# jayleicn/ClipBERT

Hardware: NVIDIA H100
Metric: clips/sec fwd+bwd MSRVTT ret (ResNet50+BERT-base) (higher is better)
Workload: dtype bf16

## Files before the change

clipbert_b200/csrc/common.cuh:

```cuda
#pragma once
#include <cuda.h>
#include <cuda_bf16.h>
#include <cuda_runtime.h>
#include <stdint.h>

#include "drop_cfg.h"

namespace cb {

#ifndef CB_SPIN_LIMIT
#define CB_SPIN_LIMIT (1u << 24)
#endif

__device__ __forceinline__ uint32_t smem_u32(const void* p) {
  return static_cast<uint32_t>(__cvta_generic_to_shared(p));
}

__device__ __forceinline__ void pdl_wait() { asm volatile("griddepcontrol.wait;" ::: "memory"); }
__device__ __forceinline__ void pdl_trigger() { asm volatile("griddepcontrol.launch_dependents;" ::: "memory"); }

__device__ __forceinline__ void mbar_init(uint64_t* bar, uint32_t count) {
  asm volatile("mbarrier.init.shared::cta.b64 [%0], %1;" ::"r"(smem_u32(bar)), "r"(count));
}
__device__ __forceinline__ void fence_mbar_init() {
// ... 94 lines not shown
  asm volatile("cp.async.bulk.wait_group.read %0;" ::"n"(N) : "memory");
}
template <int N>
__device__ __forceinline__ void tma_store_wait_all() {
  asm volatile("cp.async.bulk.wait_group %0;" ::"n"(N) : "memory");
}
__device__ __forceinline__ void named_bar_sync(uint32_t id, uint32_t nthreads) {
  asm volatile("bar.sync %0, %1;" ::"r"(id), "r"(nthreads) : "memory");
}
__device__ __forceinline__ void named_bar_arrive(uint32_t id, uint32_t nthreads) {
  asm volatile("bar.arrive %0, %1;" ::"r"(id), "r"(nthreads) : "memory");
}
template <uint32_t NREG>
__device__ __forceinline__ void setmaxnreg_dec() {
  asm volatile("setmaxnreg.dec.sync.aligned.u32 %0;" ::"n"(NREG));
}
template <uint32_t NREG>
__device__ __forceinline__ void setmaxnreg_inc() {
  asm volatile("setmaxnreg.inc.sync.aligned.u32 %0;" ::"n"(NREG));
}

__device__ __forceinline__ void wgmma_fence() { asm volatile("wgmma.fence.sync.aligned;" ::: "memory"); }
__device__ __forceinline__ void wgmma_commit() { asm volatile("wgmma.commit_group.sync.aligned;" ::: "memory"); }
template <int N>
__device__ __forceinline__ void wgmma_wait() {
  asm volatile("wgmma.wait_group.sync.aligned %0;" ::"n"(N) : "memory");
}
template <int R>
__device__ __forceinline__ void wgmma_fence_acc(float (&d)[R]) {
#pragma unroll
  for (int i = 0; i < R; ++i) asm volatile("" : "+f"(d[i])::"memory");
}

__device__ __forceinline__ uint64_t gmma_desc(uint32_t smem_addr, uint32_t lbo, uint32_t sbo) {
  uint64_t d = 0;
  d |= static_cast<uint64_t>((smem_addr & 0x3FFFFu) >> 4);
  d |= static_cast<uint64_t>((lbo >> 4) & 0x3FFFu) << 16;
  d |= static_cast<uint64_t>((sbo >> 4) & 0x3FFFu) << 32;
  d |= 1ull << 62;
  return d;
}

template <int TA, int TB>
__device__ __forceinline__ void wgmma_bf16_n64(float (&d)[32], uint64_t adesc, uint64_t bdesc, uint32_t accumulate) {
  asm volatile(
      "{\n\t.reg .pred p;\n\t"
      "setp.ne.b32 p, %34, 0;\n\t"
      "wgmma.mma_async.sync.aligned.m64n64k16.f32.bf16.bf16 "
      "{"
      "%0, %1, %2, %3, %4, %5, %6, %7, %8, %9, %10, %11, %12, %13, %14, %15, "
      "%16, %17, %18, %19, %20, %21, %22, %23, %24, %25, %26, %27, %28, %29, %30, %31"
      "}, %32, %33, p, 1, 1, %35, %36;\n\t}"
      : "+f"(d[0]), "+f"(d[1]), "+f"(d[2]), "+f"(d[3]), "+f"(d[4]), "+f"(d[5]), "+f"(d[6]), "+f"(d[7]),
        "+f"(d[8]), "+f"(d[9]), "+f"(d[10]), "+f"(d[11]), "+f"(d[12]), "+f"(d[13]), "+f"(d[14]), "+f"(d[15]),
        "+f"(d[16]), "+f"(d[17]), "+f"(d[18]), "+f"(d[19]), "+f"(d[20]), "+f"(d[21]), "+f"(d[22]), "+f"(d[23]),
        "+f"(d[24]), "+f"(d[25]), "+f"(d[26]), "+f"(d[27]), "+f"(d[28]), "+f"(d[29]), "+f"(d[30]), "+f"(d[31])
      : "l"(adesc), "l"(bdesc), "r"(accumulate), "n"(TA), "n"(TB));
}
template <int TA, int TB>
__device__ __forceinline__ void wgmma_bf16_n128(float (&d)[64], uint64_t adesc, uint64_t bdesc, uint32_t accumulate) {
  asm volatile(
      "{\n\t.reg .pred p;\n\t"
      "setp.ne.b32 p, %66, 0;\n\t"
      "wgmma.mma_async.sync.aligned.m64n128k16.f32.bf16.bf16 "
      "{"
      "%0, %1, %2, %3, %4, %5, %6, %7, %8, %9, %10, %11, %12, %13, %14, %15, "
      "%16, %17, %18, %19, %20, %21, %22, %23, %24, %25, %26, %27, %28, %29, %30, %31, "
      "%32, %33, %34, %35, %36, %37, %38, %39, %40, %41, %42, %43, %44, %45, %46, %47, "
      "%48, %49, %50, %51, %52, %53, %54, %55, %56, %57, %58, %59, %60, %61, %62, %63"
      "}, %64, %65, p, 1, 1, %67, %68;\n\t}"
      : "+f"(d[0]), "+f"(d[1]), "+f"(d[2]), "+f"(d[3]), "+f"(d[4]), "+f"(d[5]), "+f"(d[6]), "+f"(d[7]),
// ... 152 lines not shown
```

clipbert_b200/csrc/gemm.cu:

```cuda
#include <algorithm>

#include "common.cuh"
#include "host_util.h"

namespace cb {

constexpr int BM = 128;
constexpr int BK = 64;
constexpr int CONSUMER_WARPS = 8;
constexpr int GEMM_THREADS = (CONSUMER_WARPS + 1) * 32;
constexpr int PP_THREADS = 3 * 128;
constexpr int PP_PRODUCER_REGS = 40;
constexpr int PP_CONSUMER_REGS = 232;
constexpr int PP_BAR_TURN = 1;
constexpr int MAX_STAGES = 8;
constexpr int SMEM_LIMIT = 232448;
constexpr int STG_PITCH = 36;
constexpr int STG_WARP_FLOATS = 16 * STG_PITCH;
constexpr int EPI_BYTES = CONSUMER_WARPS * STG_WARP_FLOATS * 4;
constexpr int IN_BOX_BYTES = BM * 64 * 2;

struct GemmEpi {
  const float* scale;
  const float* shift;
// ... 219 lines not shown
    const int nch = min(KCH, n_iters - i);
    mbar_wait(&full_bar[s], ph);
    __syncwarp();
    wgmma_fence();
    wgmma_fence_acc(acc);
    for (int ch = 0; ch < nch; ++ch) {
      const uint32_t a_addr = smem0 + s * stage_bytes + ch * Cfg::STAGE_BYTES + wg * (64 * 128);
      const uint32_t b_addr = smem0 + s * stage_bytes + ch * Cfg::STAGE_BYTES + Cfg::A_BYTES;
#pragma unroll
      for (int k = 0; k < BK / 16; ++k) {
        const uint64_t ad = TA ? gmma_desc(a_addr + k * 2048, BK * 128, 1024) : gmma_desc(a_addr + k * 32, 16, 1024);
        const uint64_t bd = TB ? gmma_desc(b_addr + k * 2048, BK * 128, 1024) : gmma_desc(b_addr + k * 32, 16, 1024);
        wgmma_bf16<BN, TA, TB>(acc, ad, bd, (i > 0 || ch > 0 || k > 0) ? 1u : 0u);
      }
    }
    wgmma_commit();
    wgmma_wait<1>();
    wgmma_fence_acc(acc);
    if (prev >= 0) {
      __syncwarp();
      if (lane == 0) mbar_arrive(&empty_bar[prev]);
    }
    prev = s;
    if (++s == STAGES) { s = 0; ph ^= 1; }
  }
  wgmma_wait<0>();
  wgmma_fence_acc(acc);
  if (prev >= 0) {
    __syncwarp();
    if (lane == 0) mbar_arrive(&empty_bar[prev]);
  }
}

template <int BN, int TB>
__device__ __forceinline__ void mma_tile_pp(float (&acc)[2][BN / 2], uint32_t smem0, int stage_bytes, int KCH, int STAGES, int n_iters,
                                            int lane, int& s, uint32_t& ph, uint64_t* full_bar, uint64_t* empty_bar, int pass_bar,
                                            bool in_stage) {
  using Cfg = GemmCfg<BN>;
  int prev = -1;
  for (int i = 0; i < n_iters; i += KCH) {
    const int nch = min(KCH, n_iters - i);
    mbar_wait_unguarded(&full_bar[s], ph);
    __syncwarp();
    wgmma_fence();
    wgmma_fence_acc(acc[0]);
    wgmma_fence_acc(acc[1]);
    for (int ch = 0; ch < nch; ++ch) {
      const uint32_t a_addr = smem0 + s * stage_bytes + ch * Cfg::STAGE_BYTES;
      const uint32_t b_addr = a_addr + Cfg::A_BYTES;
#pragma unroll
      for (int k = 0; k < BK / 16; ++k) {
        const uint64_t bd = TB ? gmma_desc(b_addr + k * 2048, BK * 128, 1024) : gmma_desc(b_addr + k * 32, 16, 1024);
        const uint32_t accum = (i > 0 || ch > 0 || k > 0) ? 1u : 0u;
#pragma unroll
        for (int h = 0; h < 2; ++h) wgmma_bf16<BN, 0, TB>(acc[h], gmma_desc(a_addr + h * (64 * 128) + k * 32, 16, 1024), bd, accum);
      }
    }
    wgmma_commit();
    wgmma_wait<1>();
    wgmma_fence_acc(acc[0]);
    wgmma_fence_acc(acc[1]);
    if (prev >= 0) {
      __syncwarp();
      mbar_arrive_if(&empty_bar[prev], lane == 0);
    }
    prev = s;
    if (++s == STAGES) { s = 0; ph ^= 1; }
    if (pass_bar && i + KCH >= n_iters) {
      if (in_stage) mbar_wait_unguarded(&full_bar[s], ph);
      named_bar_arrive(pass_bar, 2 * 128);
    }
  }
  wgmma_wait<0>();
  wgmma_fence_acc(acc[0]);
  wgmma_fence_acc(acc[1]);
  if (prev >= 0) {
    __syncwarp();
    mbar_arrive_if(&empty_bar[prev], lane == 0);
  }
}

template <int BN, bool STORE = false>
__device__ __forceinline__ void wgrad_epilogue(const float (&acc)[BN / 2], float* obase, int64_t out_ld, const float* scale, int M, int N, int r0,
                                               int n0, int lane) {
  const int r1 = r0 + 8;
  const float rs0 = (r0 < M && scale) ? scale[r0] : 1.0f;
  const float rs1 = (r1 < M && scale) ? scale[r1] : 1.0f;
#pragma unroll
  for (int j = 0; j < BN / 8; ++j) {
    const int n = n0 + j * 8 + 2 * (lane & 3);
    if (n < N) {
      if constexpr (STORE) {
        if (r0 < M) *reinterpret_cast<float2*>(obase + static_cast<int64_t>(r0) * out_ld + n) = make_float2(acc[4 * j] * rs0, acc[4 * j + 1] * rs0);
        if (r1 < M) *reinterpret_cast<float2*>(obase + static_cast<int64_t>(r1) * out_ld + n) = make_float2(acc[4 * j + 2] * rs1, acc[4 * j + 3] * rs1);
      } else {
        if (r0 < M) red_add_f32x2(obase + static_cast<int64_t>(r0) * out_ld + n, acc[4 * j] * rs0, acc[4 * j + 1] * rs0);
        if (r1 < M) red_add_f32x2(obase + static_cast<int64_t>(r1) * out_ld + n, acc[4 * j + 2] * rs1, acc[4 * j + 3] * rs1);
      }
    }
  }
}

__device__ __forceinline__ uint32_t swz128(uint32_t box, int r, int q) { return box + r * 128 + ((q ^ (r & 7)) << 4); }

template <int BN, int MODE>
__global__ void __launch_bounds__(PP_THREADS, 1)
    gemm_pingpong_kernel(const __grid_constant__ CUtensorMap tmA, const __grid_constant__ CUtensorMap tmB, const __grid_constant__ CUtensorMap tmR,
                         const __grid_constant__ CUtensorMap tmX, int M, int N, int K, int ntaps, int tap_w, int tap_sign, int tiles_m,
                         int tiles_n, int total_tiles, int STAGES, int KCH, int N_IN, GemmEpi epi) {
  static_assert(MODE != 1 && BN <= 128, "TN / NN tiles of 128 x 64 or 128 x 128");
  using Cfg = GemmCfg<BN>;
  extern __shared__ uint8_t smem_raw[];
  uint8_t* smem = reinterpret_cast<uint8_t*>((reinterpret_cast<uintptr_t>(smem_raw) + 1023) & ~static_cast<uintptr_t>(1023));
  const int stage_bytes = KCH * Cfg::STAGE_BYTES;
  const bool has_res = epi.residual != nullptr, has_aux = epi.aux != nullptr;
  constexpr int IN_TILE_BYTES = (BN / 64) * IN_BOX_BYTES;
  const int in_bytes = (has_res + has_aux) * IN_TILE_BYTES;
  uint8_t* in_base = smem + STAGES * stage_bytes;
  uint8_t* stg_base = in_base + N_IN * in_bytes;
  uint64_t* full_bar = reinterpret_cast<uint64_t*>(stg_base + EPI_BYTES);
  uint64_t* empty_bar = full_bar + MAX_STAGES;
  uint64_t* in_full = empty_bar + MAX_STAGES;
  uint64_t* in_empty = in_full + 2;

  const int warp = __shfl_sync(0xffffffffu, static_cast<int>(threadIdx.x >> 5), 0);
  const int lane = threadIdx.x & 31;
  const int unit = blockIdx.x;
  const int n_units = gridDim.x;
  if (threadIdx.x == 0) dbg_stamp(epi, 0);
  pdl_trigger();
  if (threadIdx.x == 0) {
    tma_prefetch_desc(&tmA);
    tma_prefetch_desc(&tmB);
    if (has_res) tma_prefetch_desc(&tmR);
    if (has_aux) tma_prefetch_desc(&tmX);
    for (int s = 0; s < STAGES; ++s) {
      mbar_init(&full_bar[s], 1);
      mbar_init(&empty_bar[s], 4);
    }
    for (int b = 0; b < 2; ++b) {
      mbar_init(&in_full[b], 1);
      mbar_init(&in_empty[b], 4);
    }
    fence_mbar_init();
  }
  __syncthreads();
  const int kc_per_tap = (K + BK - 1) / BK;
  const int n_iters = ntaps * kc_per_tap;
  const bool in_stage = in_bytes && !N_IN;
  const int tile_stages = (n_iters + KCH - 1) / KCH + (in_stage ? 1 : 0);
  pdl_wait();
  if (threadIdx.x == 0) dbg_stamp(epi, 1);

  if (warp < 4) {
    setmaxnreg_dec<PP_PRODUCER_REGS>();
    if (warp == 0 && lane == 0) {
      constexpr int B_BOXES = (MODE == 0) ? 1 : BN / 64;
      int s = 0;
      uint32_t ph = 0;
      auto load_inputs = [&](int tile) {
        const TileInfo t = decode_tile<BN>(tile, tiles_m, tiles_n);
        uint64_t* bar;
        uint8_t* dst;
        if (N_IN) {
          const int local = (tile - unit) / n_units;
          const int b = N_IN == 2 ? (local & 1) : 0;
          const int uses = N_IN == 2 ? (local >> 1) : local;
          mbar_wait(&in_empty[b], (static_cast<uint32_t>(uses) & 1u) ^ 1u);
          bar = &in_full[local & 1];
          dst = in_base + b * in_bytes;
        } else {
          mbar_wait(&empty_bar[s], ph ^ 1);
          bar = &full_bar[s];
          dst = smem + s * stage_bytes;
          if (++s == STAGES) { s = 0; ph ^= 1; }
        }
        mbar_expect_tx(bar, in_bytes);
        if (has_res) {
#pragma unroll
          for (int j = 0; j < BN / 64; ++j) tma_load_2d(dst + j * IN_BOX_BYTES, &tmR, bar, t.n0 + j * 64, t.m0);
          dst += IN_TILE_BYTES;
        }
        if (has_aux) {
#pragma unroll
          for (int j = 0; j < BN / 64; ++j) tma_load_2d(dst + j * IN_BOX_BYTES, &tmX, bar, t.n0 + j * 64, t.m0);
        }
      };
      int pend = -1;
      for (int tile = unit; tile < total_tiles; tile += n_units) {
        const TileInfo t = decode_tile<BN>(tile, tiles_m, tiles_n);
        const bool inputs_first = tile < unit + N_IN * n_units;
        if (in_bytes && N_IN && inputs_first) load_inputs(tile);
        for (int i = 0; i < n_iters; i += KCH) {
          const int nch = min(KCH, n_iters - i);
          mbar_wait(&empty_bar[s], ph ^ 1);
          mbar_expect_tx(&full_bar[s], nch * Cfg::STAGE_BYTES);
          int tp = 0, kc = i;
          if (ntaps > 1) { tp = i / kc_per_tap; kc = i - tp * kc_per_tap; }
          for (int ch = 0; ch < nch; ++ch) {
            uint8_t* sa = smem + s * stage_bytes + ch * Cfg::STAGE_BYTES;
            uint8_t* sb = sa + Cfg::A_BYTES;
            int shift = 0;
            if (ntaps == 9) shift = tap_sign * ((tp / 3 - 1) * tap_w + (tp % 3 - 1));
            else if (ntaps > 1) shift = tap_sign * tp * tap_w;
            tma_load_2d(sa, &tmA, &full_bar[s], kc * BK, t.m0 + shift);
            if (MODE == 0) {
              tma_load_2d(sb, &tmB, &full_bar[s], tp * K + kc * BK, t.n0);
            } else if (epi.mn3d) {
              tma_load_3d(sb, &tmB, &full_bar[s], 0, kc * BK, (tp * N + t.n0) >> 6);
            } else {
#pragma unroll
              for (int j = 0; j < B_BOXES; ++j) tma_load_2d(sb + j * (BK * 128), &tmB, &full_bar[s], tp * N + t.n0 + j * 64, kc * BK);
            }
            if (++kc == kc_per_tap) { kc = 0; ++tp; }
          }
          if (++s == STAGES) { s = 0; ph ^= 1; }
          if (i == 0 && tile == unit) dbg_stamp(epi, 2);
        }
        if (in_stage) load_inputs(tile);
        if (pend >= 0) load_inputs(pend);
        pend = (in_bytes && N_IN && !inputs_first) ? tile : -1;
      }
      if (pend >= 0) load_inputs(pend);
      dbg_stamp(epi, 3);
    }
    return;
  }

  setmaxnreg_inc<PP_CONSUMER_REGS>();
  const int wg = (warp >> 2) - 1;
  const int wq = warp & 3;
  const uint32_t smem0 = smem_u32(smem);
  const uint64_t dseed = epi.drop_thresh ? drop_seed(epi.seed, epi.seed_off) : 0ull;
  float acc[2][BN / 2];
  int s = 0;
  uint32_t ph = 0;
  auto ring_skip = [&](int n) {
    s += n;
    while (s >= STAGES) { s -= STAGES; ph ^= 1; }
  };
  if (wg == 1) ring_skip(tile_stages);

  const int er = lane & 15, eh = lane >> 4;
  float* stg = reinterpret_cast<float*>(stg_base) + (warp - 4) * STG_WARP_FLOATS;
  const bool has_out2 = epi.out2 != nullptr;
  const bool has_shift = epi.shift != nullptr;
  const bool full = (N & 15) == 0 && epi.scale == nullptr;
  const bool drop = epi.drop_thresh != 0;
  int kind = EK_GENERIC;
  if (full) {
    if (!drop && !has_out2 && !has_aux && (epi.act == CB_ACT_NONE || epi.act == CB_ACT_RELU)) kind = EK_SHIFT_ACT;
    else if (!drop && !has_out2 && !has_shift && has_aux && epi.aux_mode == CB_AUX_RELU_MASK && epi.act == CB_ACT_NONE) kind = EK_RELU_MASK;
    else if (drop && !has_out2 && !has_aux && epi.act == CB_ACT_NONE) kind = EK_DROP_RES;
    else if (!drop && has_out2 && !has_aux && !has_res && epi.act == CB_ACT_GELU_STASH_GRAD) kind = EK_GELU_STASH;
    else if (!drop && !has_out2 && !has_shift && has_aux && epi.aux_mode == CB_AUX_MUL && epi.act == CB_ACT_NONE) kind = EK_AUX_MUL;
  }
  const bool kind_relu = epi.act == CB_ACT_RELU;
  const bool guard = (N & 15) != 0;

  for (int local = wg, tile = unit + wg * n_units; tile < total_tiles; local += 2, tile += 2 * n_units) {
    const TileInfo t = decode_tile<BN>(tile, tiles_m, tiles_n);
    if (local > 0) named_bar_sync(PP_BAR_TURN + wg, 2 * 128);
    const int pass = tile + n_units < total_tiles ? PP_BAR_TURN + (wg ^ 1) : 0;
    mma_tile_pp<BN, MODE != 0>(acc, smem0, stage_bytes, KCH, STAGES, n_iters, lane, s, ph, full_bar, empty_bar, pass, in_stage);

    const uint32_t in_buf = N_IN ? smem_u32(in_base) + (N_IN == 2 ? wg : 0) * in_bytes : smem0 + s * stage_bytes;
    if (in_bytes) {
      if (N_IN) mbar_wait_unguarded(&in_full[wg], static_cast<uint32_t>(local >> 1) & 1u);
      else mbar_wait_unguarded(&full_bar[s], ph);
    }
    int orow_half[2];
#pragma unroll
    for (int h = 0; h < 2; ++h) {
      const int m = t.m0 + h * 64 + wq * 16 + er;
      bool row_ok = m < M;
      int64_t orow = m;
      if (epi.rowmap == CB_ROWMAP_PAD) {
        const int hw = epi.H * epi.W;
        const int img = m / hw;
        const int r = m - img * hw;
        const int y = r / epi.W, x = r - y * epi.W;
        orow = (static_cast<int64_t>(img) * (epi.H + 2) + y + 1) * (epi.W + 2) + x + 1;
      } else if (epi.rowmap == CB_ROWMAP_UNPAD) {
        const int wp = epi.W + 2, hp = epi.H + 2;
        const int img = m / (hp * wp);
        const int r = m - img * (hp * wp);
        const int y = r / wp, x = r - y * wp;
        row_ok = row_ok && y >= 1 && y <= epi.H && x >= 1 && x <= epi.W;
        orow = (static_cast<int64_t>(img) * epi.H + (y - 1)) * epi.W + (x - 1);
      }
      orow_half[h] = row_ok ? static_cast<int>(orow) : -1;
    }
#pragma unroll
    for (int sc = 0; sc < BN / 32; ++sc) {
#pragma unroll 1
      for (int h = 0; h < 2; ++h) {
        const int wrow = h * 64 + wq * 16;
// ... 83 lines not shown
    }
    if (in_bytes) {
      __syncwarp();
      if (lane == 0) mbar_arrive(N_IN ? &in_empty[N_IN == 2 ? wg : 0] : &empty_bar[s]);
      if (!N_IN && ++s == STAGES) { s = 0; ph ^= 1; }
    }
    ring_skip(tile_stages);
  }
  if (threadIdx.x == 4 * 32) dbg_stamp(epi, 11);
}

static int g_sm_limit = 0;
static int sm_count_device() {
  static int n = 0;
  if (n == 0) {
    int dev = 0;
    cudaGetDevice(&dev);
    cudaDeviceGetAttribute(&n, cudaDevAttrMultiProcessorCount, dev);
    if (n <= 0) n = 132;
  }
  return n;
}
static int sm_count() {
  const int n = sm_count_device();
  return (g_sm_limit > 0 && g_sm_limit < n) ? g_sm_limit : n;
}
static int plan_sm_count() { return g_det.load(std::memory_order_relaxed) ? sm_count_device() : sm_count(); }

static long long* g_gemm_timeline = nullptr;
static int g_mn3d = 1;


struct SmemPlan {
  int epi_bytes, kch, stages, chunk_bytes, n_in;
};
static SmemPlan plan_ring(int bn, bool staging, int kiters, int force_kch, int in_bytes, int n_in) {
  SmemPlan p;
  const int limit = SMEM_LIMIT;
  p.chunk_bytes = BM * BK * 2 + bn * BK * 2;
  p.epi_bytes = staging ? EPI_BYTES : 0;
  p.n_in = n_in;
  const int chunks_fit = (limit - 1024 - GemmCfg<64>::BAR_BYTES - p.epi_bytes - n_in * in_bytes) / p.chunk_bytes;
  const int min_stages = kiters > chunks_fit ? 3 : 2;
  p.kch = 1;
  if (force_kch > 0) p.kch = force_kch;
  else if (kiters >= 4 && chunks_fit >= 4 * min_stages) p.kch = 4;
  else if (kiters >= 2 && chunks_fit >= 2 * min_stages) p.kch = 2;
  if (p.kch > kiters) p.kch = kiters;
  if (p.kch > 1 && chunks_fit / p.kch < 2) p.kch = 1;
  p.stages = chunks_fit / p.kch;
  if (p.stages > MAX_STAGES) p.stages = MAX_STAGES;
  const int stage_iters = ceil_div(kiters, p.kch);
  const int cap = staging ? 2 * stage_iters + 1 : (stage_iters + 1 > 2 ? stage_iters + 1 : 2);
  if (p.stages > cap) p.stages = cap;
  return p;
}
static SmemPlan plan_smem(int bn, bool staging, int kiters, int force_kch = 0, int in_bytes = 0) {
  const SmemPlan none = plan_ring(bn, staging, kiters, force_kch, 0, 0);
  if (in_bytes == 0) return none;
  const SmemPlan two = plan_ring(bn, staging, kiters, force_kch, in_bytes, 2);
  if (two.stages >= 2 && two.stages * two.kch >= kiters) return two;
  if (kiters > 4 && none.stages >= 2 && none.kch * none.chunk_bytes >= in_bytes) return none;
  return plan_ring(bn, staging, kiters, force_kch, in_bytes, 1);
}
static int epi_in_bytes(const cb_gemm_desc& d, int bn) {
  return d.mode == CB_GEMM_WGRAD ? 0 : ((d.residual != nullptr) + (d.aux != nullptr)) * (bn / 64) * IN_BOX_BYTES;
}

static int real_splits(int kc, int want) {
  const int sp = want < 1 ? 1 : (want > kc ? kc : want);
  return ceil_div(kc, ceil_div(kc, sp));
}

struct SplitReduceJob {
  float* out;
  const float* ws;
  int64_t out_ld;
  int M, W, S;
};
struct SplitReduce {
  int njobs;
  SplitReduceJob j[8];
};
__global__ void __launch_bounds__(256) wgrad_split_reduce_kernel(const __grid_constant__ SplitReduce r) {
  pdl_wait();
  pdl_trigger();
  const SplitReduceJob& J = r.j[blockIdx.y];
  const int w4 = J.W / 4;
  const int64_t total = static_cast<int64_t>(J.M) * w4, plane = static_cast<int64_t>(J.M) * J.W;
  for (int64_t i = static_cast<int64_t>(blockIdx.x) * 256 + threadIdx.x; i < total; i += static_cast<int64_t>(gridDim.x) * 256) {
    const int64_t m = i / w4;
    const int c = static_cast<int>(i - m * w4) * 4;
    float4* o = reinterpret_cast<float4*>(J.out + m * J.out_ld + c);
    float4 v = *o;
    const float* p = J.ws + m * J.W + c;
    for (int s = 0; s < J.S; ++s) {
      const float4 a = *reinterpret_cast<const float4*>(p + s * plane);
      v.x += a.x; v.y += a.y; v.z += a.z; v.w += a.w;
    }
    *o = v;
  }
}
static int launch_split_reduce(const SplitReduce& r, cudaStream_t stream, const char* what) {
  int64_t most = 0;
  for (int i = 0; i < r.njobs; ++i) most = std::max(most, static_cast<int64_t>(r.j[i].M) * (r.j[i].W / 4));
  const int gx = static_cast<int>(std::min<int64_t>(1024, (most + 255) / 256));
  launch_k(wgrad_split_reduce_kernel, dim3(gx, r.njobs), 256, 0, stream, r);
  return check_launch(what);
}

template <int BN, int MODE>
static int launch_gemm(const cb_gemm_desc& d, const GemmEpi& epi_in, cudaStream_t stream) {
  GemmEpi epi = epi_in;
  using Cfg = GemmCfg<BN>;
  static bool attr_set = false;
  auto kern = gemm_pingpong_kernel<BN, MODE>;
  if (!attr_set) {
    cudaError_t e = cudaFuncSetAttribute(kern, cudaFuncAttributeMaxDynamicSharedMemorySize, SMEM_LIMIT);
    if (e != cudaSuccess) {
      set_error("cudaFuncSetAttribute(smem=%d): %s", SMEM_LIMIT, cudaGetErrorString(e));
      return CB_ERR_CUDA;
    }
    attr_set = true;
  }
  alignas(64) CUtensorMap ta, tb, tr, tx;
  bool mn3d = false;
  const int tiles_m = ceil_div(d.m, BM), tiles_n = ceil_div(d.n, BN);
  const int total = tiles_m * tiles_n;
  const int kiters = ceil_div(d.k, BK) * d.ntaps;
  bool ok = get_tmap_2d(&ta, d.a, d.k, d.a_rows, d.a_ld, BK, BM);
  if (MODE == 0) {
    ok = ok && get_tmap_2d(&tb, d.b, static_cast<uint64_t>(d.k) * d.ntaps, d.b_rows, d.b_ld, BK, BN);
  } else {
    mn3d = g_mn3d && d.n % 64 == 0 &&
           get_tmap_3d_mn(&tb, d.b, static_cast<uint64_t>(d.n) * d.ntaps, d.b_rows, d.b_ld, BK, BN / 64);
    if (!mn3d) ok = ok && get_tmap_2d(&tb, d.b, static_cast<uint64_t>(d.n) * d.ntaps, d.b_rows, d.b_ld, 64, BK);
  }
  tr = ta;
  tx = ta;
  if (d.residual) ok = ok && get_tmap_2d(&tr, d.residual, d.n, d.m, d.res_ld, 64, BM);
  if (d.aux) ok = ok && get_tmap_2d(&tx, d.aux, d.n, d.m, d.aux_ld, 64, BM);
  if (!ok) return CB_ERR_CUDA;
  epi.mn3d = mn3d ? 1 : 0;
  const int units = sm_count();
  const int grid = total < units ? total : units;
  const int in_bytes = epi_in_bytes(d, BN);
  const SmemPlan sp = plan_smem(BN, true, kiters, (d.reserved >> 8) & 15, in_bytes);
  const int kch = sp.kch, stages = sp.stages;
  if (stages < 2) {
    set_error("cb_gemm: not enough shared memory for a 2-stage pipeline (BN=%d, epilogue %d B + inputs %d B)", BN, sp.epi_bytes,
              in_bytes);
    return CB_ERR_INVALID;
  }
  const int smem_bytes = stages * kch * Cfg::STAGE_BYTES + sp.n_in * in_bytes + sp.epi_bytes + Cfg::BAR_BYTES + 1024;
  launch_gemm_k(kern, grid, PP_THREADS, smem_bytes, stream, ta, tb, tr, tx, d.m, d.n, d.k, d.ntaps, d.tap_w, d.tap_sign, tiles_m,
                tiles_n, total, stages, kch, sp.n_in, epi);
  return check_launch("cb_gemm");
}

struct LaunchCfg {
  int bn, splits;
};

static LaunchCfg choose_config(const cb_gemm_desc& d, int units) {
  const int kc = ceil_div(d.k, BK);
  const bool wgrad = d.mode == CB_GEMM_WGRAD;
  const int block_n = (!wgrad && d.block_n == 256) ? 128 : d.block_n;
  static const int cand[3] = {64, 128, 256};
  LaunchCfg best = {64, 1};
  double best_cost = 1e30;
  for (int c = 0; c < 3; ++c) {
    const int bn = cand[c];
    if (block_n && bn != block_n) continue;
    if (!wgrad && bn == 256) continue;
    if (bn > 64 && d.n <= bn / 2) continue;
    const int64_t base = static_cast<int64_t>(ceil_div(d.m, BM)) * ceil_div(d.n, bn) * (wgrad ? d.ntaps : 1);
    const int max_split = wgrad ? (d.split_k > 0 ? d.split_k : (kc < 32 ? kc : 32)) : 1;
    for (int sp = (wgrad && d.split_k > 0) ? d.split_k : 1; sp <= max_split; ++sp) {
      const int ips = ceil_div(wgrad ? kc : kc * d.ntaps, sp);
      const int real_sp = wgrad ? ceil_div(kc, ips) : 1;
      const int64_t tiles = base * real_sp;
      const double rounds = static_cast<double>((tiles + units - 1) / units);
      const SmemPlan pl = plan_smem(bn, !wgrad, ips, (d.reserved >> 8) & 15, epi_in_bytes(d, bn));
      if (pl.stages < 2) continue;
      const double shallow = (pl.stages * pl.kch < 3 && ips > 2) ? 3.0 : 1.0;
      const double stage_cost = 450.0 + pl.kch * pl.chunk_bytes / 60.0;
      const double main_loop = ceil_div(ips, pl.kch) * stage_cost * shallow;
      double cost;
      if (wgrad) {
        cost = rounds * (main_loop + bn * 24.0) + 2500.0;
      } else {
        const double epi = bn * 30.0;
        const double per_tile = main_loop > 0.5 * (main_loop + epi) ? main_loop : 0.5 * (main_loop + epi);
        cost = rounds * per_tile + 0.5 * epi + 2500.0;
      }
      if (cost < best_cost) {
        best_cost = cost;
        best = {bn, real_sp};
      }
    }
  }
  return best;
}

constexpr int WG_MAX_PROBLEMS = 8;
struct WgradProblem {
  CUtensorMap tmA, tmB;
  float* out;
  const float* scale;
  int64_t out_ld;
  int M, N, K;
  int ntaps, tap_w, tap_sign;
  int iters_per_split, tiles_m, tiles_n;
  int tile_begin;
  int mn3d;
};
struct WgradGroup {
  int nprob, total_tiles;
  WgradProblem p[WG_MAX_PROBLEMS];
};
// ... 211 lines not shown
  return bytes;
}

static int check_wgrad_desc(const cb_gemm_desc& d, const char* who) {
  CB_REQUIRE(d.mode == CB_GEMM_WGRAD && d.out_fp32 == 1, "%s: not an fp32 WGRAD descriptor", who);
  CB_REQUIRE(d.a && d.b && d.out && d.m > 0 && d.n > 0 && d.k > 0, "%s: null operand / empty shape", who);
  CB_REQUIRE(d.m % 8 == 0 && d.n % 8 == 0, "%s: m, n must be multiples of 8 (got %d, %d)", who, d.m, d.n);
  CB_REQUIRE(d.out_ld % 4 == 0, "%s: out_ld must be a multiple of 4", who);
  CB_REQUIRE((reinterpret_cast<uintptr_t>(d.out) & 15) == 0, "%s: out must be 16-byte aligned", who);
  CB_REQUIRE(d.ntaps == 1 || d.ntaps == 9, "%s: ntaps must be 1 or 9 (got %d)", who, d.ntaps);
  return CB_OK;
}

static int launch_wgrad(const cb_gemm_desc* descs, int n, int bn, int splits, cudaStream_t stream, const char* what) {
  int64_t need = 0;
  if (g_det.load(std::memory_order_relaxed))
    for (int i = 0; i < n; ++i) need += wgrad_ws_bytes(descs[i], real_splits(ceil_div(descs[i].k, BK), splits));
  const cb_gemm_desc& d0 = descs[0];
  CB_REQUIRE(need == 0 || (d0.workspace != nullptr && d0.workspace_bytes >= need && (reinterpret_cast<uintptr_t>(d0.workspace) & 15) == 0),
             "%s: deterministic mode needs a 16-byte aligned workspace of %lld bytes in descs[0] (%s_workspace_bytes), got %lld", what,
             static_cast<long long>(need), what, static_cast<long long>(d0.workspace ? d0.workspace_bytes : 0));
  float* ws = static_cast<float*>(d0.workspace);
  switch (bn) {
    case 64: return need ? launch_wgrad_group<64, true>(descs, n, splits, ws, stream, what)
                         : launch_wgrad_group<64, false>(descs, n, splits, ws, stream, what);
    case 128: return need ? launch_wgrad_group<128, true>(descs, n, splits, ws, stream, what)
                          : launch_wgrad_group<128, false>(descs, n, splits, ws, stream, what);
    case 256: return need ? launch_wgrad_group<256, true>(descs, n, splits, ws, stream, what)
                          : launch_wgrad_group<256, false>(descs, n, splits, ws, stream, what);
    default: set_error("%s: block_n must be 0, 64, 128 or 256 (got %d)", what, bn); return CB_ERR_INVALID;
  }
}

}

extern "C" void cb_debug_gemm_timeline(void* device_buf) { cb::g_gemm_timeline = static_cast<long long*>(device_buf); }
extern "C" void cb_debug_gemm_mn3d(int on) { cb::g_mn3d = on ? 1 : 0; }
extern "C" void cb_debug_gemm_occ2(int, double) {}
extern "C" void cb_debug_gemm_sm_limit(int n) { cb::g_sm_limit = n > 0 ? n : 0; }

extern "C" int cb_gemm(const cb_gemm_desc* dp, void* stream_v) {
  using namespace cb;
  CB_REQUIRE(dp != nullptr, "cb_gemm: null descriptor");
  const cb_gemm_desc& d = *dp;
  cudaStream_t stream = static_cast<cudaStream_t>(stream_v);
  CB_REQUIRE(d.a && d.b && d.out, "cb_gemm: null operand pointer");
  CB_REQUIRE(d.m > 0 && d.n > 0 && d.k > 0, "cb_gemm: empty problem m=%d n=%d k=%d", d.m, d.n, d.k);
  CB_REQUIRE(d.ntaps == 1 || d.ntaps == 9 || (d.ntaps == 4 && d.mode == CB_GEMM_TN),
             "cb_gemm: ntaps must be 1, 9 (3x3 conv) or 4 (row taps, TN only) (got %d)", d.ntaps);
  CB_REQUIRE(d.mode == CB_GEMM_TN || d.mode == CB_GEMM_WGRAD || d.mode == CB_GEMM_NN, "cb_gemm: bad mode %d", d.mode);
  CB_REQUIRE(d.dropout_p >= 0.0f && d.dropout_p <= 1.0f, "cb_gemm: dropout_p %g outside [0, 1]", d.dropout_p);

  GemmEpi epi;
  epi.scale = d.scale;
  epi.shift = d.shift;
  epi.residual = static_cast<const __nv_bfloat16*>(d.residual);
  epi.aux = static_cast<const __nv_bfloat16*>(d.aux);
  epi.aux_mode = d.aux ? d.aux_mode : CB_AUX_NONE;
  epi.act = d.act;
  epi.out = d.out;
  epi.out_ld = d.out_ld;
  epi.out_fp32 = d.out_fp32;
  epi.out2 = static_cast<__nv_bfloat16*>(d.out2);
  epi.out2_ld = d.out2_ld;
  epi.rowmap = d.rowmap;
  epi.H = d.map_h;
  epi.W = d.map_w;
  epi.seed = d.dropout_seed;
  epi.dbg = g_gemm_timeline;
  epi.mn3d = 0;
  {
    const DropCfg dc = make_drop(d.dropout_p, d.dropout_seed);
// ... 72 lines not shown
```

include/clipbert_b200.h:

```cpp
#ifndef CLIPBERT_B200_H_
#define CLIPBERT_B200_H_

#include <stddef.h>
#include <stdint.h>

#ifdef __cplusplus
extern "C" {
#endif

typedef enum cb_status {
  CB_OK = 0,
  CB_ERR_INVALID = -1,
  CB_ERR_CUDA = -2,
  CB_ERR_UNSUPPORTED = -3
} cb_status;

const char* cb_last_error(void);
int cb_version(void);
int cb_sm_arch(void);
int64_t cb_launch_count(void);
int cb_set_pdl(int enable);

int cb_set_deterministic(int enable);

// ... 23 lines not shown
  int32_t m, n, k;
  const void* a;
  int64_t a_rows, a_ld;
  const void* b;
  int64_t b_rows, b_ld;
  int32_t ntaps, tap_w, tap_sign;
  int32_t split_k;
  const float* scale;
  const float* shift;
  const void* residual;
  int64_t res_ld;
  const void* aux;
  int64_t aux_ld;
  int32_t aux_mode;
  int32_t act;
  void* out;
  int64_t out_ld;
  int32_t out_fp32;
  void* out2;
  int64_t out2_ld;
  int32_t rowmap, map_h, map_w;
  float dropout_p;
  uint64_t dropout_seed;
  int32_t block_n;
  int32_t reserved;
  void* workspace;
  int64_t workspace_bytes;
} cb_gemm_desc;

int cb_gemm(const cb_gemm_desc* desc, void* stream);
int64_t cb_gemm_workspace_bytes(const cb_gemm_desc* desc);
int cb_gemm_wgrad_group(const cb_gemm_desc* descs, int n, void* stream);
int64_t cb_gemm_wgrad_group_workspace_bytes(const cb_gemm_desc* descs, int n);

int cb_layernorm_fwd(const void* x, const float* gamma, const float* beta, void* y, float* stats, int m, int hidden,
                     float eps, void* stream);
int cb_layernorm_bwd(const void* dy, const void* x, const float* stats, const float* gamma, void* dx, void* dx_drop,
                     float* dgamma, float* dbeta, float* dbias_drop, int m, int hidden, float dropout_p,
                     uint64_t dropout_seed, void* stream);
int64_t cb_layernorm_bwd_scratch_bytes(int m);
int cb_layernorm_bwd_det(const void* dy, const void* x, const float* stats, const float* gamma, void* dx, void* dx_drop,
                         float* dgamma, float* dbeta, float* dbias_drop, int m, int hidden, float dropout_p,
                         uint64_t dropout_seed, float* scratch, int64_t scratch_bytes, void* stream);

int cb_embed_text_fwd(const int64_t* ids, const float* word, const float* pos, const float* type0, const float* gamma,
                      const float* beta, void* out, float* stats, int nseq, int lt, int l, int vocab, int hidden,
                      float eps, float dropout_p, uint64_t seed, void* stream);
int cb_embed_text_bwd(const void* dh, const int64_t* ids, const float* word, const float* pos, const float* type0,
                      const float* gamma, const float* stats, float* dword, float* dpos, float* dtype0, float* dgamma,
                      float* dbeta, int nseq, int lt, int l, int vocab, int hidden, float dropout_p, uint64_t seed,
                      void* stream);
int cb_embed_visual_fwd(const void* grid, const int32_t* seq2vid, int n_ex, const float* rowemb, const float* colemb,
                        const float* type0, const float* gamma, const float* beta, void* out, float* stats, int nseq,
                        int t, int gh, int gw, int lt, int l, int hidden, float eps, float dropout_p, uint64_t seed,
                        void* stream);
int cb_embed_visual_bwd(const void* dh, const void* grid, const int32_t* seq2vid, const int32_t* vid_start, int n_ex,
                        const float* rowemb, const float* colemb, const float* type0, const float* gamma,
                        const float* stats, float* dv_tmp, void* dgrid, float* drow, float* dcol, float* dtype0,
                        float* dgamma, float* dbeta, int nseq, int nvid, int t, int gh, int gw, int lt, int l, int hidden,
                        float dropout_p, uint64_t seed, void* stream);
int64_t cb_embed_text_bwd_scratch_bytes(int nseq, int lt);
int cb_embed_text_bwd_det(const void* dh, const int64_t* ids, const float* word, const float* pos, const float* type0,
                          const float* gamma, const float* stats, float* dword, float* dpos, float* dtype0, float* dgamma,
                          float* dbeta, int nseq, int lt, int l, int vocab, int hidden, float dropout_p, uint64_t seed,
                          float* scratch, int64_t scratch_bytes, void* stream);
int64_t cb_embed_visual_bwd_scratch_bytes(int nseq, int gh, int gw);
// ... 66 lines not shown
```

Measured before the change: 3984.

## Reuse a shared-memory halo slab across the nine taps of 3x3 conv GEMMs

For 3x3 implicit-GEMM convolutions in the TN ping-pong kernel, each output tile now loads the activation rows plus a halo once into a double-buffered shared-memory slab. All nine taps then read their A operand by offsetting the wgmma descriptor into that slab, instead of reloading a shifted A tile per tap through the stage ring. This is meant to cut TMA and L2 traffic and shrink each ring stage to B only. In exchange the slab takes shared memory and pipeline depth, and the path depends on 128B-swizzle descriptors staying valid at arbitrary row offsets. The planner falls back to the old path when fewer than three stages fit, and a debug kernel is added to check swizzle row-phase behaviour.

After: 3984 (median of 6 runs). Within noise of the previous version (-0.0%).

```diff
diff --git a/clipbert_b200/csrc/common.cuh b/clipbert_b200/csrc/common.cuh
--- a/clipbert_b200/csrc/common.cuh
+++ b/clipbert_b200/csrc/common.cuh
@@ -150,11 +150,12 @@
   for (int i = 0; i < R; ++i) asm volatile("" : "+f"(d[i])::"memory");
 }
 
-__device__ __forceinline__ uint64_t gmma_desc(uint32_t smem_addr, uint32_t lbo, uint32_t sbo) {
+__device__ __forceinline__ uint64_t gmma_desc(uint32_t smem_addr, uint32_t lbo, uint32_t sbo, uint32_t base_offset = 0) {
   uint64_t d = 0;
   d |= static_cast<uint64_t>((smem_addr & 0x3FFFFu) >> 4);
   d |= static_cast<uint64_t>((lbo >> 4) & 0x3FFFu) << 16;
   d |= static_cast<uint64_t>((sbo >> 4) & 0x3FFFu) << 32;
+  d |= static_cast<uint64_t>(base_offset & 7u) << 49;
   d |= 1ull << 62;
   return d;
 }
diff --git a/clipbert_b200/csrc/gemm.cu b/clipbert_b200/csrc/gemm.cu
--- a/clipbert_b200/csrc/gemm.cu
+++ b/clipbert_b200/csrc/gemm.cu
@@ -275,12 +275,14 @@
   }
 }
 
-template <int BN, int TB>
-__device__ __forceinline__ void mma_tile_pp(float (&acc)[2][BN / 2], uint32_t smem0, int stage_bytes, int KCH, int STAGES, int n_iters,
-                                            int lane, int& s, uint32_t& ph, uint64_t* full_bar, uint64_t* empty_bar, int pass_bar,
-                                            bool in_stage) {
+template <int BN, int TB, bool SLAB>
+__device__ __forceinline__ void mma_tile_pp(float (&acc)[2][BN / 2], uint32_t smem0, int stage_bytes, int chunk_bytes, int KCH, int STAGES,
+                                            int n_iters, int lane, int& s, uint32_t& ph, uint64_t* full_bar, uint64_t* empty_bar,
+                                            int pass_bar, bool in_stage, uint32_t slab, int slab_pitch, int kc_per_tap, int tap_w,
+                                            int tap_sign) {
   using Cfg = GemmCfg<BN>;
   int prev = -1;
+  int tp = 0, kc = 0;
   for (int i = 0; i < n_iters; i += KCH) {
     const int nch = min(KCH, n_iters - i);
     mbar_wait_unguarded(&full_bar[s], ph);
@@ -289,8 +291,13 @@
     wgmma_fence_acc(acc[0]);
     wgmma_fence_acc(acc[1]);
     for (int ch = 0; ch < nch; ++ch) {
-      const uint32_t a_addr = smem0 + s * stage_bytes + ch * Cfg::STAGE_BYTES;
-      const uint32_t b_addr = a_addr + Cfg::A_BYTES;
+      uint32_t a_addr = smem0 + s * stage_bytes + ch * chunk_bytes;
+      uint32_t b_addr = a_addr + Cfg::A_BYTES;
+      if constexpr (SLAB) {
+        b_addr = a_addr;
+        a_addr = slab + kc * slab_pitch + (tap_sign * ((tp / 3 - 1) * tap_w + (tp % 3 - 1)) + tap_w + 1) * 128;
+        if (++kc == kc_per_tap) { kc = 0; ++tp; }
+      }
 #pragma unroll
       for (int k = 0; k < BK / 16; ++k) {
         const uint64_t bd = TB ? gmma_desc(b_addr + k * 2048, BK * 128, 1024) : gmma_desc(b_addr + k * 32, 16, 1024);
@@ -346,25 +353,32 @@
 
 __device__ __forceinline__ uint32_t swz128(uint32_t box, int r, int q) { return box + r * 128 + ((q ^ (r & 7)) << 4); }
 
-template <int BN, int MODE>
+template <int BN, int MODE, bool SLAB>
 __global__ void __launch_bounds__(PP_THREADS, 1)
     gemm_pingpong_kernel(const __grid_constant__ CUtensorMap tmA, const __grid_constant__ CUtensorMap tmB, const __grid_constant__ CUtensorMap tmR,
                          const __grid_constant__ CUtensorMap tmX, int M, int N, int K, int ntaps, int tap_w, int tap_sign, int tiles_m,
-                         int tiles_n, int total_tiles, int STAGES, int KCH, int N_IN, GemmEpi epi) {
+                         int tiles_n, int total_tiles, int STAGES, int KCH, int N_IN, int slab_rows, int slab_box_rows, GemmEpi epi) {
   static_assert(MODE != 1 && BN <= 128, "TN / NN tiles of 128 x 64 or 128 x 128");
   using Cfg = GemmCfg<BN>;
   extern __shared__ uint8_t smem_raw[];
   uint8_t* smem = reinterpret_cast<uint8_t*>((reinterpret_cast<uintptr_t>(smem_raw) + 1023) & ~static_cast<uintptr_t>(1023));
-  const int stage_bytes = KCH * Cfg::STAGE_BYTES;
+  const int chunk_bytes = SLAB ? Cfg::B_BYTES : Cfg::STAGE_BYTES;
+  const int stage_bytes = KCH * chunk_bytes;
+  const int kc_per_tap = (K + BK - 1) / BK;
+  const int slab_pitch = SLAB ? slab_rows * 128 : 0;
+  const int slab_bytes = kc_per_tap * slab_pitch;
   const bool has_res = epi.residual != nullptr, has_aux = epi.aux != nullptr;
   constexpr int IN_TILE_BYTES = (BN / 64) * IN_BOX_BYTES;
   const int in_bytes = (has_res + has_aux) * IN_TILE_BYTES;
-  uint8_t* in_base = smem + STAGES * stage_bytes;
+  uint8_t* slab_base = smem + STAGES * stage_bytes;
+  uint8_t* in_base = slab_base + 2 * slab_bytes;
   uint8_t* stg_base = in_base + N_IN * in_bytes;
   uint64_t* full_bar = reinterpret_cast<uint64_t*>(stg_base + EPI_BYTES);
   uint64_t* empty_bar = full_bar + MAX_STAGES;
   uint64_t* in_full = empty_bar + MAX_STAGES;
   uint64_t* in_empty = in_full + 2;
+  uint64_t* slab_full = in_empty + 2;
+  uint64_t* slab_empty = slab_full + 2;
 
   const int warp = __shfl_sync(0xffffffffu, static_cast<int>(threadIdx.x >> 5), 0);
   const int lane = threadIdx.x & 31;
@@ -384,11 +398,12 @@
     for (int b = 0; b < 2; ++b) {
       mbar_init(&in_full[b], 1);
       mbar_init(&in_empty[b], 4);
+      mbar_init(&slab_full[b], 1);
+      mbar_init(&slab_empty[b], 4);
     }
     fence_mbar_init();
   }
   __syncthreads();
-  const int kc_per_tap = (K + BK - 1) / BK;
   const int n_iters = ntaps * kc_per_tap;
   const bool in_stage = in_bytes && !N_IN;
   const int tile_stages = (n_iters + KCH - 1) / KCH + (in_stage ? 1 : 0);
@@ -429,6 +444,18 @@
           for (int j = 0; j < BN / 64; ++j) tma_load_2d(dst + j * IN_BOX_BYTES, &tmX, bar, t.n0 + j * 64, t.m0);
         }
       };
+      auto load_slab = [&](int tile) {
+        const int local = (tile - unit) / n_units;
+        const int b = local & 1;
+        mbar_wait(&slab_empty[b], (static_cast<uint32_t>(local >> 1) & 1u) ^ 1u);
+        mbar_expect_tx(&slab_full[b], slab_bytes);
+        const int r0 = decode_tile<BN>(tile, tiles_m, tiles_n).m0 - (tap_w + 1);
+        uint8_t* dst = slab_base + b * slab_bytes;
+        for (int kc = 0; kc < kc_per_tap; ++kc)
+          for (int r = 0; r < slab_rows; r += slab_box_rows) tma_load_2d(dst + kc * slab_pitch + r * 128, &tmA, &slab_full[b], kc * BK, r0 + r);
+      };
+      const int slab_at = min(STAGES, (n_iters + KCH - 1) / KCH) - 1;
+      if (SLAB && unit < total_tiles) load_slab(unit);
       int pend = -1;
       for (int tile = unit; tile < total_tiles; tile += n_units) {
         const TileInfo t = decode_tile<BN>(tile, tiles_m, tiles_n);
@@ -437,16 +464,18 @@
         for (int i = 0; i < n_iters; i += KCH) {
           const int nch = min(KCH, n_iters - i);
           mbar_wait(&empty_bar[s], ph ^ 1);
-          mbar_expect_tx(&full_bar[s], nch * Cfg::STAGE_BYTES);
+          mbar_expect_tx(&full_bar[s], nch * chunk_bytes);
           int tp = 0, kc = i;
           if (ntaps > 1) { tp = i / kc_per_tap; kc = i - tp * kc_per_tap; }
           for (int ch = 0; ch < nch; ++ch) {
-            uint8_t* sa = smem + s * stage_bytes + ch * Cfg::STAGE_BYTES;
-            uint8_t* sb = sa + Cfg::A_BYTES;
-            int shift = 0;
-            if (ntaps == 9) shift = tap_sign * ((tp / 3 - 1) * tap_w + (tp % 3 - 1));
-            else if (ntaps > 1) shift = tap_sign * tp * tap_w;
-            tma_load_2d(sa, &tmA, &full_bar[s], kc * BK, t.m0 + shift);
+            uint8_t* sb = smem + s * stage_bytes + ch * chunk_bytes;
+            if (!SLAB) {
+              int shift = 0;
+              if (ntaps == 9) shift = tap_sign * ((tp / 3 - 1) * tap_w + (tp % 3 - 1));
+              else if (ntaps > 1) shift = tap_sign * tp * tap_w;
+              tma_load_2d(sb, &tmA, &full_bar[s], kc * BK, t.m0 + shift);
+              sb += Cfg::A_BYTES;
+            }
             if (MODE == 0) {
               tma_load_2d(sb, &tmB, &full_bar[s], tp * K + kc * BK, t.n0);
             } else if (epi.mn3d) {
@@ -459,6 +488,7 @@
           }
           if (++s == STAGES) { s = 0; ph ^= 1; }
           if (i == 0 && tile == unit) dbg_stamp(epi, 2);
+          if (SLAB && i == slab_at * KCH && tile + n_units < total_tiles) load_slab(tile + n_units);
         }
         if (in_stage) load_inputs(tile);
         if (pend >= 0) load_inputs(pend);
@@ -505,7 +535,13 @@
     const TileInfo t = decode_tile<BN>(tile, tiles_m, tiles_n);
     if (local > 0) named_bar_sync(PP_BAR_TURN + wg, 2 * 128);
     const int pass = tile + n_units < total_tiles ? PP_BAR_TURN + (wg ^ 1) : 0;
-    mma_tile_pp<BN, MODE != 0>(acc, smem0, stage_bytes, KCH, STAGES, n_iters, lane, s, ph, full_bar, empty_bar, pass, in_stage);
+    if (SLAB) mbar_wait_unguarded(&slab_full[wg], static_cast<uint32_t>(local >> 1) & 1u);
+    mma_tile_pp<BN, MODE != 0, SLAB>(acc, smem0, stage_bytes, chunk_bytes, KCH, STAGES, n_iters, lane, s, ph, full_bar, empty_bar, pass, in_stage,
+                               smem_u32(slab_base) + wg * slab_bytes, slab_pitch, kc_per_tap, tap_w, tap_sign);
+    if (SLAB) {
+      __syncwarp();
+      mbar_arrive_if(&slab_empty[wg], lane == 0);
+    }
 
     const uint32_t in_buf = N_IN ? smem_u32(in_base) + (N_IN == 2 ? wg : 0) * in_bytes : smem0 + s * stage_bytes;
     if (in_bytes) {
@@ -655,15 +691,16 @@
 
 
 struct SmemPlan {
-  int epi_bytes, kch, stages, chunk_bytes, n_in;
+  int epi_bytes, kch, stages, chunk_bytes, n_in, slab_bytes;
 };
-static SmemPlan plan_ring(int bn, bool staging, int kiters, int force_kch, int in_bytes, int n_in) {
+static SmemPlan plan_ring(int bn, bool staging, int kiters, int force_kch, int in_bytes, int n_in, int slab_bytes) {
   SmemPlan p;
   const int limit = SMEM_LIMIT;
-  p.chunk_bytes = BM * BK * 2 + bn * BK * 2;
+  p.chunk_bytes = (slab_bytes ? 0 : BM * BK * 2) + bn * BK * 2;
   p.epi_bytes = staging ? EPI_BYTES : 0;
   p.n_in = n_in;
-  const int chunks_fit = (limit - 1024 - GemmCfg<64>::BAR_BYTES - p.epi_bytes - n_in * in_bytes) / p.chunk_bytes;
+  p.slab_bytes = slab_bytes;
+  const int chunks_fit = (limit - 1024 - GemmCfg<64>::BAR_BYTES - p.epi_bytes - n_in * in_bytes - 2 * slab_bytes) / p.chunk_bytes;
   const int min_stages = kiters > chunks_fit ? 3 : 2;
   p.kch = 1;
   if (force_kch > 0) p.kch = force_kch;
@@ -678,16 +715,41 @@
   if (p.stages > cap) p.stages = cap;
   return p;
 }
-static SmemPlan plan_smem(int bn, bool staging, int kiters, int force_kch = 0, int in_bytes = 0) {
-  const SmemPlan none = plan_ring(bn, staging, kiters, force_kch, 0, 0);
+static SmemPlan plan_smem(int bn, bool staging, int kiters, int force_kch = 0, int in_bytes = 0, int slab_bytes = 0) {
+  const SmemPlan none = plan_ring(bn, staging, kiters, force_kch, 0, 0, slab_bytes);
   if (in_bytes == 0) return none;
-  const SmemPlan two = plan_ring(bn, staging, kiters, force_kch, in_bytes, 2);
+  const SmemPlan two = plan_ring(bn, staging, kiters, force_kch, in_bytes, 2, slab_bytes);
   if (two.stages >= 2 && two.stages * two.kch >= kiters) return two;
   if (kiters > 4 && none.stages >= 2 && none.kch * none.chunk_bytes >= in_bytes) return none;
-  return plan_ring(bn, staging, kiters, force_kch, in_bytes, 1);
+  return plan_ring(bn, staging, kiters, force_kch, in_bytes, 1, slab_bytes);
 }
 static int epi_in_bytes(const cb_gemm_desc& d, int bn) {
   return d.mode == CB_GEMM_WGRAD ? 0 : ((d.residual != nullptr) + (d.aux != nullptr)) * (bn / 64) * IN_BOX_BYTES;
+}
+
+constexpr int CB_RESERVED_PER_TAP = 1 << 12;
+
+struct SlabPlan {
+  int rows, box_rows, bytes;
+};
+static SlabPlan conv_slab(const cb_gemm_desc& d) {
+  SlabPlan s = {0, 0, 0};
+  if (d.mode == CB_GEMM_WGRAD || d.ntaps != 9 || (d.reserved & CB_RESERVED_PER_TAP)) return s;
+  const int rows = BM + 2 * (d.tap_w + 1);
+  const int boxes = ceil_div(rows, 256);
+  s.box_rows = ceil_div(ceil_div(rows, boxes), 8) * 8;
+  s.rows = boxes * s.box_rows;
+  s.bytes = ceil_div(d.k, BK) * s.rows * 128;
+  return s;
+}
+static SmemPlan plan_tn(const cb_gemm_desc& d, int bn) {
+  const int kiters = ceil_div(d.k, BK) * d.ntaps, force_kch = (d.reserved >> 8) & 15, in_bytes = epi_in_bytes(d, bn);
+  const SlabPlan slab = conv_slab(d);
+  if (slab.bytes) {
+    const SmemPlan p = plan_smem(bn, true, kiters, force_kch, in_bytes, slab.bytes);
+    if (p.stages >= 3) return p;
+  }
+  return plan_smem(bn, true, kiters, force_kch, in_bytes);
 }
 
 static int real_splits(int kc, int want) {
@@ -737,12 +799,13 @@
   GemmEpi epi = epi_in;
   using Cfg = GemmCfg<BN>;
   static bool attr_set = false;
-  auto kern = gemm_pingpong_kernel<BN, MODE>;
   if (!attr_set) {
-    cudaError_t e = cudaFuncSetAttribute(kern, cudaFuncAttributeMaxDynamicSharedMemorySize, SMEM_LIMIT);
-    if (e != cudaSuccess) {
-      set_error("cudaFuncSetAttribute(smem=%d): %s", SMEM_LIMIT, cudaGetErrorString(e));
-      return CB_ERR_CUDA;
+    for (auto k : {gemm_pingpong_kernel<BN, MODE, false>, gemm_pingpong_kernel<BN, MODE, true>}) {
+      cudaError_t e = cudaFuncSetAttribute(k, cudaFuncAttributeMaxDynamicSharedMemorySize, SMEM_LIMIT);
+      if (e != cudaSuccess) {
+        set_error("cudaFuncSetAttribute(smem=%d): %s", SMEM_LIMIT, cudaGetErrorString(e));
+        return CB_ERR_CUDA;
+      }
     }
     attr_set = true;
   }
@@ -750,8 +813,10 @@
   bool mn3d = false;
   const int tiles_m = ceil_div(d.m, BM), tiles_n = ceil_div(d.n, BN);
   const int total = tiles_m * tiles_n;
-  const int kiters = ceil_div(d.k, BK) * d.ntaps;
-  bool ok = get_tmap_2d(&ta, d.a, d.k, d.a_rows, d.a_ld, BK, BM);
+  const int in_bytes = epi_in_bytes(d, BN);
+  const SmemPlan sp = plan_tn(d, BN);
+  const SlabPlan slab = sp.slab_bytes ? conv_slab(d) : SlabPlan{0, 0, 0};
+  bool ok = get_tmap_2d(&ta, d.a, d.k, d.a_rows, d.a_ld, BK, slab.bytes ? slab.box_rows : BM);
   if (MODE == 0) {
     ok = ok && get_tmap_2d(&tb, d.b, static_cast<uint64_t>(d.k) * d.ntaps, d.b_rows, d.b_ld, BK, BN);
   } else {
@@ -767,17 +832,15 @@
   epi.mn3d = mn3d ? 1 : 0;
   const int units = sm_count();
   const int grid = total < units ? total : units;
-  const int in_bytes = epi_in_bytes(d, BN);
-  const SmemPlan sp = plan_smem(BN, true, kiters, (d.reserved >> 8) & 15, in_bytes);
   const int kch = sp.kch, stages = sp.stages;
   if (stages < 2) {
     set_error("cb_gemm: not enough shared memory for a 2-stage pipeline (BN=%d, epilogue %d B + inputs %d B)", BN, sp.epi_bytes,
               in_bytes);
     return CB_ERR_INVALID;
   }
-  const int smem_bytes = stages * kch * Cfg::STAGE_BYTES + sp.n_in * in_bytes + sp.epi_bytes + Cfg::BAR_BYTES + 1024;
-  launch_gemm_k(kern, grid, PP_THREADS, smem_bytes, stream, ta, tb, tr, tx, d.m, d.n, d.k, d.ntaps, d.tap_w, d.tap_sign, tiles_m,
-                tiles_n, total, stages, kch, sp.n_in, epi);
+  const int smem_bytes = stages * kch * sp.chunk_bytes + 2 * sp.slab_bytes + sp.n_in * in_bytes + sp.epi_bytes + Cfg::BAR_BYTES + 1024;
+  launch_gemm_k(slab.bytes ? gemm_pingpong_kernel<BN, MODE, true> : gemm_pingpong_kernel<BN, MODE, false>, grid, PP_THREADS, smem_bytes, stream, ta, tb, tr, tx, d.m, d.n, d.k, d.ntaps, d.tap_w, d.tap_sign, tiles_m,
+                tiles_n, total, stages, kch, sp.n_in, slab.rows, slab.box_rows, epi);
   return check_launch("cb_gemm");
 }
 
@@ -804,11 +867,11 @@
       const int real_sp = wgrad ? ceil_div(kc, ips) : 1;
       const int64_t tiles = base * real_sp;
       const double rounds = static_cast<double>((tiles + units - 1) / units);
-      const SmemPlan pl = plan_smem(bn, !wgrad, ips, (d.reserved >> 8) & 15, epi_in_bytes(d, bn));
+      const SmemPlan pl = wgrad ? plan_smem(bn, false, ips, (d.reserved >> 8) & 15) : plan_tn(d, bn);
       if (pl.stages < 2) continue;
       const double shallow = (pl.stages * pl.kch < 3 && ips > 2) ? 3.0 : 1.0;
       const double stage_cost = 450.0 + pl.kch * pl.chunk_bytes / 60.0;
-      const double main_loop = ceil_div(ips, pl.kch) * stage_cost * shallow;
+      const double main_loop = ceil_div(ips, pl.kch) * stage_cost * shallow + pl.slab_bytes / 60.0;
       double cost;
       if (wgrad) {
         cost = rounds * (main_loop + bn * 24.0) + 2500.0;
@@ -1086,12 +1149,70 @@
   }
 }
 
+__global__ void __launch_bounds__(128, 1)
+    sw128_row_phase_kernel(const __grid_constant__ CUtensorMap tmSlab, const __grid_constant__ CUtensorMap tmRows,
+                           const __grid_constant__ CUtensorMap tmB, float* out) {
+  extern __shared__ uint8_t smem_raw[];
+  uint8_t* slab = reinterpret_cast<uint8_t*>((reinterpret_cast<uintptr_t>(smem_raw) + 1023) & ~static_cast<uintptr_t>(1023));
+  uint8_t* b = slab + 10 * 1024;
+  uint8_t* rows = b + 8 * 1024;
+  __shared__ uint64_t bar;
+  pdl_wait();
+  if (threadIdx.x == 0) {
+    mbar_init(&bar, 1);
+    fence_mbar_init();
+    mbar_expect_tx(&bar, 72 * 128 + 8192 + 8 * 8192);
+    tma_load_2d(slab, &tmSlab, &bar, 0, 0);
+    tma_load_2d(b, &tmB, &bar, 0, 0);
+    for (int p = 0; p < 8; ++p) tma_load_2d(rows + p * 8192, &tmRows, &bar, 0, p);
+  }
+  __syncthreads();
+  mbar_wait(&bar, 0);
+#pragma unroll 1
+  for (int pv = 0; pv < 24; ++pv) {
+    const int p = pv / 3, v = pv % 3;
+    const uint32_t a0 = v == 2 ? smem_u32(rows + p * 8192) : smem_u32(slab) + p * 128;
+    float acc[32];
+    wgmma_fence();
+#pragma unroll
+    for (int k = 0; k < BK / 16; ++k)
+      wgmma_bf16<64, 0, 0>(acc, gmma_desc(a0 + k * 32, 16, 1024, v == 1 ? (a0 >> 7) & 7 : 0), gmma_desc(smem_u32(b) + k * 32, 16, 1024),
+                           k > 0 ? 1u : 0u);
+    wgmma_commit();
+    wgmma_wait<0>();
+    wgmma_fence_acc(acc);
+    float* o = out + (pv * 128 + threadIdx.x) * 32;
+#pragma unroll
+    for (int j = 0; j < 32; ++j) o[j] = acc[j];
+  }
+}
+
 }
 
 extern "C" void cb_debug_gemm_timeline(void* device_buf) { cb::g_gemm_timeline = static_cast<long long*>(device_buf); }
 extern "C" void cb_debug_gemm_mn3d(int on) { cb::g_mn3d = on ? 1 : 0; }
 extern "C" void cb_debug_gemm_occ2(int, double) {}
 extern "C" void cb_debug_gemm_sm_limit(int n) { cb::g_sm_limit = n > 0 ? n : 0; }
+extern "C" int cb_debug_gemm_plan(const cb_gemm_desc* d, int* slab) {
+  using namespace cb;
+  const LaunchCfg lc = choose_config(*d, sm_count());
+  *slab = plan_tn(*d, lc.bn).slab_bytes > 0 ? 1 : 0;
+  return lc.bn;
+}
+extern "C" int cb_debug_sw128_row_phase(const void* a, const void* b, float* out, void* stream) {
+  using namespace cb;
+  alignas(64) CUtensorMap ts, tr, tb;
+  if (!(get_tmap_2d(&ts, a, 64, 72, 64, 64, 72) && get_tmap_2d(&tr, a, 64, 72, 64, 64, 64) && get_tmap_2d(&tb, b, 64, 64, 64, 64, 64)))
+    return CB_ERR_CUDA;
+  const int smem = 1024 + 18 * 1024 + 8 * 8192;
+  cudaError_t e = cudaFuncSetAttribute(sw128_row_phase_kernel, cudaFuncAttributeMaxDynamicSharedMemorySize, smem);
+  if (e != cudaSuccess) {
+    set_error("cudaFuncSetAttribute(smem=%d): %s", smem, cudaGetErrorString(e));
+    return CB_ERR_CUDA;
+  }
+  launch_k(sw128_row_phase_kernel, dim3(1), dim3(128), smem, static_cast<cudaStream_t>(stream), ts, tr, tb, out);
+  return check_launch("cb_debug_sw128_row_phase");
+}
 
 extern "C" int cb_gemm(const cb_gemm_desc* dp, void* stream_v) {
   using namespace cb;
diff --git a/include/clipbert_b200.h b/include/clipbert_b200.h
--- a/include/clipbert_b200.h
+++ b/include/clipbert_b200.h
@@ -79,6 +79,8 @@
 int64_t cb_gemm_workspace_bytes(const cb_gemm_desc* desc);
 int cb_gemm_wgrad_group(const cb_gemm_desc* descs, int n, void* stream);
 int64_t cb_gemm_wgrad_group_workspace_bytes(const cb_gemm_desc* descs, int n);
+int cb_debug_gemm_plan(const cb_gemm_desc* desc, int* slab);
+int cb_debug_sw128_row_phase(const void* a, const void* b, float* out, void* stream);
 
 int cb_layernorm_fwd(const void* x, const float* gamma, const float* beta, void* y, float* stats, int m, int hidden,
                      float eps, void* stream);
```
